# msotoodeh/curve25519

Measured on AMD Instinct MI355X. Metric: X25519 shared-key ops/sec (batch=2^20 per GPU, variable-base Montgomery ladder) [+ Ed25519 verifies/sec in `verify`], higher is better.
Workload: dtype u64

## Files before the change

### curve25519_amd/csrc/engine_verify.hip

```cpp
#include "engine_common.cuh"
#include "verify_check.cuh"

constexpr int FS_BLOCK = 256;
#ifndef C25519_VW_WAVES
#define C25519_VW_WAVES 2
#endif
#ifndef C25519_WALK_BLOCK
#define C25519_WALK_BLOCK C25519_ED_BLOCK
#endif
constexpr int WALK_BLOCK = C25519_WALK_BLOCK;
#ifndef C25519_VD_WAVES
#define C25519_VD_WAVES 3
#endif

template <bool Strict = false>
C25519_DEV void verify_scalars_lane(const FastScratch& fs, const void* sig, const void* pk, const Msgs& msgs, size_t n, size_t i)
{
    u32 pkw[8], Rw[8], Sw[8], cols[SIGMA_WORDS], rho[5], tau[5], tau_neg;
    load32(pkw, pk, i);
    load32(Rw, sig, 2 * i);
    load32(Sw, sig, 2 * i + 1);
    const u32 lat_ok = ed_verify_fast_scalars(cols, rho, tau, tau_neg, pkw, Rw, Sw, msgs.ptr(i), msgs.len(i), fs.lat_cap_bits);
#pragma unroll
    for (int w = 0; w < SIGMA_WORDS; w++) fs.sigma[(size_t)w * n + i] = cols[w];
#pragma unroll
    for (int w = 0; w < 5; w++) { fs.rho[(size_t)w * n + i] = rho[w]; fs.tau[(size_t)w * n + i] = tau[w]; }
    const int top = lat_ok ? walk_top_digit(tau, rho) : 0;
    if (Strict) {
        load32(Rw, sig, 2 * i);
        load32(Sw, sig, 2 * i + 1);
        fs.flags[i] = (lat_ok & FLAG_FITS) | (tau_neg & FLAG_TAU_NEG) | ((u32)top << 8) | strict_pair_flags(Rw, Sw);
    } else
        fs.flags[i] = (lat_ok & FLAG_FITS) | (tau_neg & FLAG_TAU_NEG) | ((u32)top << 8);
}


template <bool Strict>
C25519_DEV void verify_fast_scalars(const FastScratch& fs, const void* sig, const void* pk, const Msgs& msgs, size_t n)
{
    const size_t i = (size_t)blockIdx.x * FS_BLOCK + threadIdx.x;
    if (i == 0) fs.slow_count[0] = fs.slow_count[1] = fs.slow_count[2] = 0;
    if (i >= n) return;
    verify_scalars_lane<Strict>(fs, sig, pk, msgs, n, i);
}

__global__ void __launch_bounds__(FS_BLOCK) k_ed25519_verify_fast_scalars(FastScratch fs, const void* sig, const void* pk,
                                                                          Msgs msgs, size_t n)
{
    verify_fast_scalars<false>(fs, sig, pk, msgs, n);
}

__global__ void __launch_bounds__(FS_BLOCK) k_ed25519_verify_fast_scalars_strict(FastScratch fs, const void* sig, const void* pk,
                                                                                 Msgs msgs, size_t n)
{
    verify_fast_scalars<true>(fs, sig, pk, msgs, n);
}

template <bool Strict>
C25519_DEV void verify_fast_points(FastScratch fs, const void* sig, const void* pk, size_t n, int* verdict)
{
    const size_t j = (size_t)blockIdx.x * ED_BLOCK + threadIdx.x;
    if (j >= 2 * n) return;
    const bool is_r = j >= n;
    const size_t e = is_r ? j - n : j;
    u32 w[8];
    if (is_r) load32(w, sig, 2 * e); else load32(w, pk, e);
    const u32 f = fs.flags[e];
    const u32 tau_neg = (f & FLAG_TAU_NEG) ? 0xffffffffu : 0u;
    fe X, Y;
    const u32 ok = ed_verify_fast_decode(X, Y, w, is_r ? 0xffffffffu : 0u, tau_neg) & (Strict && !is_r ? ~strict_reject_key(w) : 0xffffffffu);
    if (!is_r) {
        const bool is_long = ((f >> 8) & 63u) > 32u;
        const u32 pos = is_long ? (u32)n - 1u - atomicAdd(fs.slow_count + 2, 1u) : atomicAdd(fs.slow_count + 1, 1u);
        fs.order[pos] = (u32)e;
    }
    if (is_r) {
        if (ok) atomicOr(&fs.flags[e], FLAG_R_OK);
    } else if (Strict) {
        const u32 add = strict_key_flags(f, ok);
        atomicOr(&fs.flags[e], add);
        if (add & FLAG_REJECT) verdict[e] = 0;
        else if (add & FLAG_SLOW) fs.slow_list[atomicAdd(fs.slow_count, 1u)] = (u32)e;
    } else if (ok && (f & FLAG_FITS)) {
        atomicOr(&fs.flags[e], FLAG_KEY_OK);
    } else {
        atomicOr(&fs.flags[e], ok ? FLAG_KEY_OK | FLAG_SLOW : FLAG_SLOW);
        fs.slow_list[atomicAdd(fs.slow_count, 1u)] = (u32)e;
    }
    wtable_build(fs.tables + e * FAST_TABLE_WORDS + (is_r ? WTABLE_WORDS : 0), X, Y);
}

__global__ void __launch_bounds__(ED_BLOCK, C25519_VD_WAVES) k_ed25519_verify_fast_points(FastScratch fs, const void* sig, const void* pk,
                                                                                          size_t n)
{
    verify_fast_points<false>(fs, sig, pk, n, nullptr);
}

__global__ void __launch_bounds__(ED_BLOCK, C25519_VD_WAVES) k_ed25519_verify_fast_points_strict(FastScratch fs, const void* sig,
                                                                                                 const void* pk, size_t n, int* verdict)
{
    verify_fast_points<true>(fs, sig, pk, n, verdict);
}

__global__ void __launch_bounds__(WALK_BLOCK, C25519_VW_WAVES) k_ed25519_verify_fast_walk(FastScratch fs, int* verdict, size_t n,
                                                                                        const u32* __restrict__ g_tbl)
{
    __shared__ __attribute__((aligned(16))) u32 lds_tbl[SC_TBL_WORDS];
    lds_stage_words(lds_tbl, g_tbl + SC_TBL_OFFSET, SC_TBL_WORDS);
    const size_t lane = (size_t)blockIdx.x * WALK_BLOCK + threadIdx.x;
    const size_t i = lane < n ? fs.order[lane] : n;
    const u32 f = i < n ? fs.flags[i] : FLAG_SLOW;
    const bool walks = !(f & FLAG_SLOW);
    int top = walks ? (int)((f >> 8) & 63u) : 0;
#pragma unroll
    for (int o = 32; o >= 1; o >>= 1) {
        const int other = __shfl_xor(top, o);
        top = other > top ? other : top;
    }
    top = __builtin_amdgcn_readfirstlane(top);
    if (!walks) return;
    const u32* tq = fs.tables + i * FAST_TABLE_WORDS;
    const WalkScalars sc{ fs.sigma, fs.tau, fs.rho, n, i };
    const u32 neutral = ge_walk_is_neutral(sc, tq, tq + WTABLE_WORDS, lds_tbl, top < 8 ? 8 : top);
    verdict[i] = (neutral & f & FLAG_R_OK) ? 1 : 0;
}

__global__ void __launch_bounds__(ED_BLOCK, C25519_VD_WAVES) k_ed25519_verify_quad_prep(FastScratch fs, const void* sig, const void* pk,
                                                                                         Msgs msgs, size_t n, unsigned scalar_blocks)
{
    static_assert(FS_BLOCK == ED_BLOCK, "one workgroup shape for both roles");
    if (blockIdx.x < scalar_blocks) {
        const size_t i = (size_t)blockIdx.x * FS_BLOCK + threadIdx.x;
        if (i == 0) fs.slow_count[0] = fs.slow_count[1] = fs.slow_count[2] = 0;
        if (i >= n) return;
        verify_scalars_lane(fs, sig, pk, msgs, n, i);
        return;
    }
    const size_t j = (size_t)(blockIdx.x - scalar_blocks) * ED_BLOCK + threadIdx.x;
    if (j >= 2 * n) return;
    const bool is_r = j >= n;
    const size_t e = is_r ? j - n : j;
    u32 w[8];
    if (is_r) load32(w, sig, 2 * e); else load32(w, pk, e);
    fe X, Y;
    const u32 ok = ed_verify_fast_decode(X, Y, w, is_r ? 0xffffffffu : 0u, 0u);
    fs.pflags[j] = ok;
    wtable_build(fs.tables + e * FAST_TABLE_WORDS + (is_r ? WTABLE_WORDS : 0), X, Y);
}

__global__ void __launch_bounds__(ED_BLOCK, C25519_VD_WAVES) k_ed25519_verify_quad_prep_strict(FastScratch fs, const void* sig, const void* pk,
                                                                                                Msgs msgs, size_t n, unsigned scalar_blocks)
{
    if (blockIdx.x < scalar_blocks) {
        const size_t i = (size_t)blockIdx.x * FS_BLOCK + threadIdx.x;
        if (i == 0) fs.slow_count[0] = fs.slow_count[1] = fs.slow_count[2] = 0;
        if (i >= n) return;
        verify_scalars_lane<true>(fs, sig, pk, msgs, n, i);
        return;
    }
    const size_t j = (size_t)(blockIdx.x - scalar_blocks) * ED_BLOCK + threadIdx.x;
    if (j >= 2 * n) return;
    const bool is_r = j >= n;
    const size_t e = is_r ? j - n : j;
    u32 w[8];
    if (is_r) load32(w, sig, 2 * e); else load32(w, pk, e);
    fe X, Y;
    const u32 ok = ed_verify_fast_decode(X, Y, w, is_r ? 0xffffffffu : 0u, 0u) & (is_r ? 0xffffffffu : ~strict_reject_key(w));
    fs.pflags[j] = ok;
    wtable_build(fs.tables + e * FAST_TABLE_WORDS + (is_r ? WTABLE_WORDS : 0), X, Y);
}

constexpr int QW_BLOCK = 256;
__global__ void __launch_bounds__(QW_BLOCK) __attribute__((amdgpu_waves_per_eu(1, 2)))
k_ed25519_verify_quad_walk(FastScratch fs, int* verdict, size_t n, const u32* __restrict__ g_tbl)
{
    __shared__ __attribute__((aligned(16))) u32 lds_tbl[SC_TBL_WORDS];
    lds_stage_words(lds_tbl, g_tbl + SC_TBL_OFFSET, SC_TBL_WORDS);
    const size_t i = (size_t)blockIdx.x * (QW_BLOCK / 4) + (threadIdx.x >> 2);
    const u32 f = i < n ? fs.flags[i] : 0u;
    const u32 key_ok = i < n ? fs.pflags[i] : 0u, r_ok = i < n ? fs.pflags[n + i] : 0u;
    const bool walks = (f & FLAG_FITS) && key_ok;
    int top = walks ? (int)((f >> 8) & 63u) : 0;
#pragma unroll
    for (int o = 32; o >= 1; o >>= 1) {
        const int other = __shfl_xor(top, o);
        top = other > top ? other : top;
    }
    top = __builtin_amdgcn_readfirstlane(top);
    const quad::Roles R = quad::roles();
    if (!walks) {
        if (i < n && R.is0) fs.slow_list[atomicAdd(fs.slow_count, 1u)] = (u32)i;
        return;
    }
    const u32* tq = fs.tables + i * FAST_TABLE_WORDS;
    const WalkScalars sc{ fs.sigma, fs.tau, fs.rho, n, i };
    const u32 q_flip = (f & FLAG_TAU_NEG) ? 0xffffffffu : 0u;
    const u32 neutral = quad::walk_is_neutral(sc, tq, tq + WTABLE_WORDS, lds_tbl, top < 8 ? 8 : top, R, q_flip);
    if (R.is0) verdict[i] = (neutral & r_ok) ? 1 : 0;
}

__global__ void __launch_bounds__(QW_BLOCK) __attribute__((amdgpu_waves_per_eu(1, 2)))
k_ed25519_verify_quad_walk_strict(FastScratch fs, int* verdict, size_t n, const u32* __restrict__ g_tbl)
{
    __shared__ __attribute__((aligned(16))) u32 lds_tbl[SC_TBL_WORDS];
    lds_stage_words(lds_tbl, g_tbl + SC_TBL_OFFSET, SC_TBL_WORDS);
    const size_t i = (size_t)blockIdx.x * (QW_BLOCK / 4) + (threadIdx.x >> 2);
    const u32 f = i < n ? fs.flags[i] : 0u;
    const u32 key_ok = i < n ? fs.pflags[i] : 0u, r_ok = i < n ? fs.pflags[n + i] : 0u;
    const bool rejected = i < n && ((f & FLAG_REJECT) || !key_ok);
    const bool walks = !rejected && (f & FLAG_FITS);
    int top = walks ? (int)((f >> 8) & 63u) : 0;
#pragma unroll
    for (int o = 32; o >= 1; o >>= 1) {
        const int other = __shfl_xor(top, o);
        top = other > top ? other : top;
    }
    top = __builtin_amdgcn_readfirstlane(top);
    const quad::Roles R = quad::roles();
    if (!walks) {
        if (rejected && R.is0) verdict[i] = 0;
        else if (i < n && R.is0) fs.slow_list[atomicAdd(fs.slow_count, 1u)] = (u32)i;
        return;
    }
    const u32* tq = fs.tables + i * FAST_TABLE_WORDS;
    const WalkScalars sc{ fs.sigma, fs.tau, fs.rho, n, i };
    const u32 q_flip = (f & FLAG_TAU_NEG) ? 0xffffffffu : 0u;
    const u32 neutral = quad::walk_is_neutral(sc, tq, tq + WTABLE_WORDS, lds_tbl, top < 8 ? 8 : top, R, q_flip);
    if (R.is0) verdict[i] = (neutral & r_ok) ? 1 : 0;
}

__global__ void __launch_bounds__(192) __attribute__((amdgpu_waves_per_eu(1, 2)))
k_ed25519_verify_one_per_group(FastScratch fs, int* verdict, const void* sig, const void* pk, Msgs msgs, size_t n,
                               const u32* __restrict__ g_tbl)
{
    __shared__ __attribute__((aligned(16))) u32 lds_all[coop::V3_LDS_WORDS];
    __shared__ u32 park[40], hand[4];
    if (blockIdx.x >= n) return;
    coop::verify_three_waves(lds_all, park, hand, fs, verdict, sig, pk, msgs, n, blockIdx.x, g_tbl);
}

__global__ void __launch_bounds__(192) __attribute__((amdgpu_waves_per_eu(1, 2)))
k_ed25519_verify_one_per_group_strict(FastScratch fs, int* verdict, const void* sig, const void* pk, Msgs msgs, size_t n,
                                      const u32* __restrict__ g_tbl)
{
    __shared__ __attribute__((aligned(16))) u32 lds_all[coop::V3_LDS_WORDS];
    __shared__ u32 park[40], hand[4];
    if (blockIdx.x >= n) return;
    coop::verify_three_waves<true>(lds_all, park, hand, fs, verdict, sig, pk, msgs, n, blockIdx.x, g_tbl);
}

__global__ void __launch_bounds__(ED_BLOCK, 2) k_ed25519_verify_slow(FastScratch fs, int* verdict, const void* sig, const void* pk,
                                                                     Msgs msgs, const u32* __restrict__ g_tbl, DoneWord done)
{
    const u32 count = *fs.slow_count;
    if (blockIdx.x == 0 && threadIdx.x == 0) {
        *fs.slow_report = count;
        if (count == 0) signal_done(done);
    }
    if ((size_t)blockIdx.x * ED_BLOCK >= count) return;
    __shared__ __attribute__((aligned(16))) u32 lds_tbl[PA_WORDS * 256];
    lds_stage_words(lds_tbl, g_tbl + REF_TBL_OFFSET, REF_TBL_WORDS);
    const size_t k = (size_t)blockIdx.x * ED_BLOCK + threadIdx.x;
    if (k >= count) return;
    const size_t i = fs.slow_list[k];
    u32 pkw[8], Rw[8], Sw[8];
    load32(pkw, pk, i);
    load32(Rw, sig, 2 * i);
    load32(Sw, sig, 2 * i + 1);
    verdict[i] = ed_verify_reference_order(pkw, Rw, Sw, msgs.ptr(i), msgs.len(i), fs.tables + i * FAST_TABLE_WORDS, lds_tbl);
    if (k == 0) signal_done(done);
}


template <bool Scale8>
C25519_DEV void verify_scalars_lane_zip215(const FastScratch& fs, const void* sig, const void* pk, const Msgs& msgs, size_t n, size_t i)
{
    u32 pkw[8], Rw[8], Sw[8], cols[SIGMA_WORDS], rho[5], tau[5], tau_neg;
    load32(pkw, pk, i);
    load32(Rw, sig, 2 * i);
    load32(Sw, sig, 2 * i + 1);
    const u32 lat_ok = ed_verify_zip215_scalars(cols, rho, tau, tau_neg, pkw, Rw, Sw, msgs.ptr(i), msgs.len(i), fs.lat_cap_bits, Scale8);
#pragma unroll
    for (int w = 0; w < SIGMA_WORDS; w++) fs.sigma[(size_t)w * n + i] = cols[w];
#pragma unroll
    for (int w = 0; w < 5; w++) { fs.rho[(size_t)w * n + i] = rho[w]; fs.tau[(size_t)w * n + i] = tau[w]; }
    const int top = lat_ok ? walk_top_digit(tau, rho) : 0;
    load32(Sw, sig, 2 * i + 1);
    fs.flags[i] = (lat_ok & FLAG_FITS) | (tau_neg & FLAG_TAU_NEG) | ((u32)top << 8) | zip215_pair_flags(Sw);
}

__global__ void __launch_bounds__(FS_BLOCK) k_ed25519_verify_fast_scalars_zip215(FastScratch fs, const void* sig, const void* pk,
                                                                                 Msgs msgs, size_t n)
{
    const size_t i = (size_t)blockIdx.x * FS_BLOCK + threadIdx.x;
    if (i == 0) fs.slow_count[0] = fs.slow_count[1] = fs.slow_count[2] = 0;
    if (i >= n) return;
    verify_scalars_lane_zip215<true>(fs, sig, pk, msgs, n, i);
}

__global__ void __launch_bounds__(ED_BLOCK, C25519_VD_WAVES) k_ed25519_verify_fast_points_zip215(FastScratch fs, const void* sig,
                                                                                                 const void* pk, size_t n, int* verdict)
{
    const size_t j = (size_t)blockIdx.x * ED_BLOCK + threadIdx.x;
    if (j >= 2 * n) return;
    const bool is_r = j >= n;
    const size_t e = is_r ? j - n : j;
    u32 w[8];
    if (is_r) load32(w, sig, 2 * e); else load32(w, pk, e);
    const u32 f = fs.flags[e];
    fe X, Y;
    const u32 ok = ed_zip215_decode(X, Y, w, (is_r || !(f & FLAG_TAU_NEG)) ? 0xffffffffu : 0u);
    if (!is_r) {
        const bool is_long = ((f >> 8) & 63u) > 33u;
        const u32 pos = is_long ? (u32)n - 1u - atomicAdd(fs.slow_count + 2, 1u) : atomicAdd(fs.slow_count + 1, 1u);
        fs.order[pos] = (u32)e;
    }
    if (is_r) {
        if (ok) atomicOr(&fs.flags[e], FLAG_R_OK);
    } else {
        const u32 add = strict_key_flags(f, ok);
        atomicOr(&fs.flags[e], add);
        if (add & FLAG_REJECT) verdict[e] = 0;
        else if (add & FLAG_SLOW) fs.slow_list[atomicAdd(fs.slow_count, 1u)] = (u32)e;
    }
    wtable_build(fs.tables + e * FAST_TABLE_WORDS + (is_r ? WTABLE_WORDS : 0), X, Y);
}

__global__ void __launch_bounds__(ED_BLOCK, C25519_VD_WAVES) k_ed25519_verify_quad_prep_zip215(FastScratch fs, const void* sig, const void* pk,
                                                                                                Msgs msgs, size_t n, unsigned scalar_blocks)
{
    if (blockIdx.x < scalar_blocks) {
        const size_t i = (size_t)blockIdx.x * FS_BLOCK + threadIdx.x;
        if (i == 0) fs.slow_count[0] = fs.slow_count[1] = fs.slow_count[2] = 0;
        if (i >= n) return;
        verify_scalars_lane_zip215<false>(fs, sig, pk, msgs, n, i);
        return;
    }
    const size_t j = (size_t)(blockIdx.x - scalar_blocks) * ED_BLOCK + threadIdx.x;
    if (j >= 2 * n) return;
    const bool is_r = j >= n;
    const size_t e = is_r ? j - n : j;
    u32 w[8];
    if (is_r) load32(w, sig, 2 * e); else load32(w, pk, e);
    fe X, Y;
    const u32 ok = ed_zip215_decode(X, Y, w, 0xffffffffu);
    fs.pflags[j] = ok;
    wtable_build(fs.tables + e * FAST_TABLE_WORDS + (is_r ? WTABLE_WORDS : 0), X, Y);
}

__global__ void __launch_bounds__(QW_BLOCK) __attribute__((amdgpu_waves_per_eu(1, 2)))
k_ed25519_verify_quad_walk_zip215(FastScratch fs, int* verdict, size_t n, const u32* __restrict__ g_tbl)
{
    __shared__ __attribute__((aligned(16))) u32 lds_tbl[SC_TBL_WORDS];
    lds_stage_words(lds_tbl, g_tbl + SC_TBL_OFFSET, SC_TBL_WORDS);
    const size_t i = (size_t)blockIdx.x * (QW_BLOCK / 4) + (threadIdx.x >> 2);
    const u32 f = i < n ? fs.flags[i] : 0u;
    const u32 key_ok = i < n ? fs.pflags[i] : 0u, r_ok = i < n ? fs.pflags[n + i] : 0u;
    const bool rejected = i < n && ((f & FLAG_REJECT) || !key_ok || !r_ok);
    const bool walks = !rejected && (f & FLAG_FITS);
    int top = walks ? (int)((f >> 8) & 63u) : 0;
#pragma unroll
    for (int o = 32; o >= 1; o >>= 1) {
        const int other = __shfl_xor(top, o);
        top = other > top ? other : top;
    }
    top = __builtin_amdgcn_readfirstlane(top);
    const quad::Roles R = quad::roles();
    if (!walks) {
        if (rejected && R.is0) verdict[i] = 0;
        else if (i < n && R.is0) fs.slow_list[atomicAdd(fs.slow_count, 1u)] = (u32)i;
        return;
    }
    const u32* tq = fs.tables + i * FAST_TABLE_WORDS;
    const WalkScalars sc{ fs.sigma, fs.tau, fs.rho, n, i };
    const u32 q_flip = (f & FLAG_TAU_NEG) ? 0xffffffffu : 0u;
    const u32 neutral = quad::walk_is_neutral<true>(sc, tq, tq + WTABLE_WORDS, lds_tbl, top < 8 ? 8 : top, R, q_flip);
    if (R.is0) verdict[i] = neutral ? 1 : 0;
}

__global__ void __launch_bounds__(192) __attribute__((amdgpu_waves_per_eu(1, 2)))
k_ed25519_verify_one_per_group_zip215(FastScratch fs, int* verdict, const void* sig, const void* pk, Msgs msgs, size_t n,
                                      const u32* __restrict__ g_tbl)
{
    __shared__ __attribute__((aligned(16))) u32 lds_all[coop::V3_LDS_WORDS];
    __shared__ u32 park[40], hand[4];
    if (blockIdx.x >= n) return;
    coop::verify_three_waves<false, true>(lds_all, park, hand, fs, verdict, sig, pk, msgs, n, blockIdx.x, g_tbl);
}

__global__ void __launch_bounds__(ED_BLOCK, 2) k_ed25519_verify_slow_zip215(FastScratch fs, int* verdict, const void* sig, const void* pk,
                                                                            Msgs msgs, const u32* __restrict__ g_tbl, DoneWord done)
{
    const u32 count = *fs.slow_count;
    if (blockIdx.x == 0 && threadIdx.x == 0) {
        *fs.slow_report = count;
        if (count == 0) signal_done(done);
    }
    if ((size_t)blockIdx.x * ED_BLOCK >= count) return;
    __shared__ __attribute__((aligned(16))) u32 lds_tbl[PA_WORDS * 256];
    lds_stage_words(lds_tbl, g_tbl + REF_TBL_OFFSET, REF_TBL_WORDS);
    const size_t k = (size_t)blockIdx.x * ED_BLOCK + threadIdx.x;
    if (k >= count) return;
    const size_t i = fs.slow_list[k];
    u32 pkw[8], Rw[8], Sw[8];
    load32(pkw, pk, i);
    load32(Rw, sig, 2 * i);
    load32(Sw, sig, 2 * i + 1);
    verdict[i] = ed_verify_zip215_reference_order(pkw, Rw, Sw, msgs.ptr(i), msgs.len(i), fs.tables + i * FAST_TABLE_WORDS, lds_tbl);
    if (k == 0) signal_done(done);
}

namespace {

constexpr size_t VERIFY_TABLE_WORDS = FAST_TABLE_WORDS > QTABLE_LIMB_WORDS ? FAST_TABLE_WORDS : QTABLE_LIMB_WORDS;
static_assert(FAST_TABLE_WORDS % 32 == 0 && VERIFY_TABLE_WORDS % 32 == 0, "per-lane tables must keep their rows 128-byte aligned");
inline size_t verify_scalar_words(size_t n) { return round_up(SIGMA_WORDS * n, 4) + 2 * round_up(5 * n, 4) + 5 * round_up(n, 4) + 4; }
inline size_t verify_scratch_bytes(size_t n)
{
    return (n * VERIFY_TABLE_WORDS + proj_words(n) + verify_scalar_words(n)) * sizeof(u32);
}

struct LastVerify { const u32* count = nullptr; hipStream_t stream = nullptr; int device = -1; unsigned long generation = 0; };
thread_local LastVerify tl_last_verify;

template <typename MakeFin>
int verify_run(const void* sig, const void* pk, Msgs msgs, size_t n, hipStream_t stream, int* verdict, bool fast, MakeFin make_fin,
               VerifyRules rules = RULES_PLAIN, bool last_in_call = true)
{
    const bool strict = rules == RULES_STRICT, zip215 = rules == RULES_ZIP215;
    const u32* tbl = nullptr;
    C25519_RC(base_tables(&tbl, nullptr));
    void* w = nullptr;
    c25519_host::WorkLease lease;
    C25519_RC(lease.acquire(&w, verify_scratch_bytes(n), stream));
    u32* tables = (u32*)w;
    const ProjScratch scr = carve_proj(tables + n * VERIFY_TABLE_WORDS, n);
    const unsigned grid = grid_for(n, ED_BLOCK);
    if (fast) {
        unsigned* report = nullptr;
        C25519_RC(tls().report_word_for(&report, stream));
        FastScratch fs;
        fs.tables = tables;
        fs.sigma = tables + n * VERIFY_TABLE_WORDS + proj_words(n);
        fs.rho = fs.sigma + round_up(SIGMA_WORDS * n, 4);
        fs.tau = fs.rho + round_up(5 * n, 4);
        fs.flags = fs.tau + round_up(5 * n, 4);
        fs.slow_list = fs.flags + round_up(n, 4);
        fs.order = fs.slow_list + round_up(n, 4);
        fs.slow_count = fs.order + round_up(n, 4);
        fs.pflags = fs.slow_count + 4;
        fs.slow_report = report;
        {
            const long cap = c25519_host::tunable_or(c25519_host::T_VERIFY_LAT_CAP_BITS, LAT_CAP_BITS);
            fs.lat_cap_bits = cap >= 100 && cap < LAT_CAP_BITS ? (int)cap : LAT_CAP_BITS;
        }
        if (!verify_quad_for(n) && verify_coop_for(n)) {
            C25519_TRY(hipMemsetAsync(fs.slow_count, 0, 3 * sizeof(u32), stream));
            note_shape(SHAPE_PER_GROUP, 192);
            (zip215 ? k_ed25519_verify_one_per_group_zip215 : strict ? k_ed25519_verify_one_per_group_strict : k_ed25519_verify_one_per_group)<<<(unsigned)n, 192, 0, stream>>>(
                fs, verdict, sig, pk, msgs, n, tbl);
            C25519_TRY(hipGetLastError());
        } else if (verify_quad_for(n)) {
            const unsigned sb = grid_for(n, FS_BLOCK);
            note_shape(SHAPE_QUAD, QW_BLOCK);
            (zip215 ? k_ed25519_verify_quad_prep_zip215 : strict ? k_ed25519_verify_quad_prep_strict : k_ed25519_verify_quad_prep)<<<sb + grid_for(2 * n, ED_BLOCK), ED_BLOCK, 0, stream>>>(
                fs, sig, pk, msgs, n, sb);
            C25519_TRY(hipGetLastError());
            (zip215 ? k_ed25519_verify_quad_walk_zip215 : strict ? k_ed25519_verify_quad_walk_strict : k_ed25519_verify_quad_walk)<<<grid_for(n, QW_BLOCK / 4), QW_BLOCK, 0, stream>>>(
                fs, verdict, n, tbl);
            C25519_TRY(hipGetLastError());
        } else {
            note_shape(SHAPE_LANE, WALK_BLOCK);
            (zip215 ? k_ed25519_verify_fast_scalars_zip215 : strict ? k_ed25519_verify_fast_scalars_strict : k_ed25519_verify_fast_scalars)<<<grid_for(n, FS_BLOCK), FS_BLOCK, 0, stream>>>(
                fs, sig, pk, msgs, n);
            C25519_TRY(hipGetLastError());
            if (zip215)
                k_ed25519_verify_fast_points_zip215<<<grid_for(2 * n, ED_BLOCK), ED_BLOCK, 0, stream>>>(fs, sig, pk, n, verdict);
            else if (strict)
                k_ed25519_verify_fast_points_strict<<<grid_for(2 * n, ED_BLOCK), ED_BLOCK, 0, stream>>>(fs, sig, pk, n, verdict);
            else
                k_ed25519_verify_fast_points<<<grid_for(2 * n, ED_BLOCK), ED_BLOCK, 0, stream>>>(fs, sig, pk, n);
            C25519_TRY(hipGetLastError());
            k_ed25519_verify_fast_walk<<<grid_for(n, WALK_BLOCK), WALK_BLOCK, 0, stream>>>(fs, verdict, n, tbl);
            C25519_TRY(hipGetLastError());
        }
        (zip215 ? k_ed25519_verify_slow_zip215 : k_ed25519_verify_slow)<<<grid, ED_BLOCK, 0, stream>>>(fs, verdict, sig, pk, msgs, tbl,
                                                                                                     last_in_call ? take_done_word(n) : DoneWord{ nullptr, 0 });
        C25519_TRY(hipGetLastError());
        tl_last_verify.count = report; tl_last_verify.stream = stream;
        tl_last_verify.generation = tls().generation;
        (void)hipGetDevice(&tl_last_verify.device);
        return lease.release();
    }
    tl_last_verify = LastVerify();
    note_shape(SHAPE_LANE_INVERT, ED_BLOCK);
    k_ed25519_verify_init<QTableLimbs><<<grid, ED_BLOCK, 0, stream>>>(pk, n, tables, VERIFY_TABLE_WORDS);
    C25519_TRY(hipGetLastError());
    k_ed25519_verify_check<QTableLimbs><<<grid, ED_BLOCK, 0, stream>>>(scr, sig, pk, msgs, n, tbl, tables, VERIFY_TABLE_WORDS);
    C25519_TRY(hipGetLastError());
    C25519_RC(launch_invert(scr, n, make_fin(scr), stream));
    return lease.release();
}

}

int c25519_engine::verify_dev(void* verdict, const void* sig, const void* pk, Msgs msgs, size_t n, hipStream_t stream, VerifyRules rules,
                              bool last_in_call)
{
    const bool fast = rules != RULES_PLAIN || c25519_host::tunable_or(c25519_host::T_VERIFY_REFERENCE_ORDER, 0) == 0;
    if (int rc = check_dev_args(n, { verdict, sig, pk })) return rc;
    if (n == 0) return 0;
    return verify_run(sig, pk, msgs, n, stream, (int*)verdict, fast,
                      [&](const ProjScratch& scr) { return FinishVerify{ scr.a, scr.b, sig, (int*)verdict, n, nullptr }; }, rules, last_in_call);
}

extern "C" {

size_t ed25519_VerifySignature_scratch_bytes(size_t n) { return verify_scratch_bytes(n); }

int c25519_amd_verify_point_dev(void* out, const void* sig, const void* pk, const void* msg, size_t msg_size, size_t n,
                                void* stream)
{
    C25519_API_CALL();
    if (!out || !sig || !pk || (!msg && msg_size)) return bad_arg("null pointer");
    if (int rc = check_dev_args(n, { out, sig, pk })) return rc;
    if (n == 0) return 0;
    return verify_run(sig, pk, fixed_msgs(msg, msg_size), n, (hipStream_t)stream, nullptr, false,
                      [&](const ProjScratch& scr) { return FinishPack{ scr.a, scr.b, out, n, 1, 0, nullptr, 0, 0 }; });
}

long c25519_amd_verify_last_slow_elements(void)
{
    C25519_API_CALL_OR(-1);
    const LastVerify& lv = tl_last_verify;
    int dev = -1;
    if (!lv.count || hipGetDevice(&dev) != hipSuccess || dev != lv.device) return -1;
    if (lv.generation != tls().generation) return -1;
    if (hipStreamSynchronize(lv.stream) != hipSuccess) return -1;
    u32 c = 0;
    if (hipMemcpy(&c, lv.count, sizeof c, hipMemcpyDeviceToHost) != hipSuccess) return -1;
    return (long)c;
}

int ed25519_VerifySignature_dev(void* verdict, const void* sig, const void* pk, const void* msg, size_t msg_size,
                                size_t n, void* stream)
{
    C25519_API_CALL();
    if (!verdict || !sig || !pk || (!msg && msg_size)) return bad_arg("null pointer");
    return verify_dev(verdict, sig, pk, fixed_msgs(msg, msg_size), n, (hipStream_t)stream, RULES_PLAIN);
}

int ed25519_VerifySignature_ragged_dev(void* verdict, const void* sig, const void* pk, const void* msgs,
                                       const uint64_t* offsets, size_t n, void* stream)
{
    C25519_API_CALL();
    if (!verdict || !sig || !pk || !offsets) return bad_arg("null pointer");
    return verify_dev(verdict, sig, pk, ragged_msgs(msgs, offsets), n, (hipStream_t)stream, RULES_PLAIN);
}

int ed25519_VerifySignature_strict_dev(void* verdict, const void* sig, const void* pk, const void* msg, size_t msg_size,
                                       size_t n, void* stream)
{
    C25519_API_CALL();
    if (!verdict || !sig || !pk || (!msg && msg_size)) return bad_arg("null pointer");
    return verify_dev(verdict, sig, pk, fixed_msgs(msg, msg_size), n, (hipStream_t)stream, RULES_STRICT);
}

int ed25519_VerifySignature_strict_ragged_dev(void* verdict, const void* sig, const void* pk, const void* msgs,
                                              const uint64_t* offsets, size_t n, void* stream)
{
    C25519_API_CALL();
    if (!verdict || !sig || !pk || !offsets) return bad_arg("null pointer");
    return verify_dev(verdict, sig, pk, ragged_msgs(msgs, offsets), n, (hipStream_t)stream, RULES_STRICT);
}

int ed25519_VerifySignature_zip215_dev(void* verdict, const void* sig, const void* pk, const void* msg, size_t msg_size,
                                       size_t n, void* stream)
{
    C25519_API_CALL();
    if (!verdict || !sig || !pk || (!msg && msg_size)) return bad_arg("null pointer");
    return verify_dev(verdict, sig, pk, fixed_msgs(msg, msg_size), n, (hipStream_t)stream, RULES_ZIP215);
}

int ed25519_VerifySignature_zip215_ragged_dev(void* verdict, const void* sig, const void* pk, const void* msgs,
                                              const uint64_t* offsets, size_t n, void* stream)
{
    C25519_API_CALL();
    if (!verdict || !sig || !pk || !offsets) return bad_arg("null pointer");
    return verify_dev(verdict, sig, pk, ragged_msgs(msgs, offsets), n, (hipStream_t)stream, RULES_ZIP215);
}

}
```

### curve25519_amd/csrc/verify_fast.cuh

```cuda
#pragma once
#include "ge25519.cuh"
#include "lanes.cuh"
#include "sc25519.cuh"
#include "sha512.cuh"

namespace c25519 {

constexpr int LAT_CAP_BITS = 158;
#ifndef C25519_LAT_COUNT
#define C25519_LAT_COUNT(what)
#endif
constexpr int LAT_LEHMER_STOP = 128;
constexpr int LAT_R = 8, LAT_T = 6;

template <int W>
C25519_DEV int bitlen_words(const u32 (&a)[W])
{
    int n = 0;
#pragma unroll
    for (int i = 0; i < W; i++) n = a[i] ? 32 * i + (32 - __builtin_clz(a[i])) : n;
    return n;
}
C25519_DEV int bitlen64(u64 x) { return x ? 64 - __builtin_clzll(x) : 0; }
template <int W>
// ... 490 lines not shown
    for (int i = 0; i < 10; i++) q.v[i] = p_ymx[i * SC_ROWS];
    fe_mul(a, a, q);
    fe_add(b, S.Y, S.X);
#pragma unroll
    for (int i = 0; i < 10; i++) q.v[i] = p_ypx[i * SC_ROWS];
    fe_mul(b, b, q);
    fe_sub(e, b, a);
    fe_add(h, b, a);
#pragma unroll
    for (int i = 0; i < 10; i++) q.v[i] = tbl[(20 + i) * SC_ROWS + r];
    fe_neg(a, q);
    fe_select(q, neg, a, q);
    fe_mul(a, S.T, q);
    fe_add(b, S.Z, S.Z);
    fe_sub(f, b, a);
    fe_add(g, b, a);
    fe_mul(S.X, f, e);
    if (need_t) fe_mul(S.T, e, h);
    fe_mul(S.Z, f, g);
    fe_mul(S.Y, g, h);
}

C25519_DEV void ge_store_pe_row(u32* row, const ge_ext& S)
{
    fe t, a;
    fe_add(t, S.Y, S.X);  fe_carry32(a, t);  store_field(row, a);
    fe_sub(t, S.Y, S.X);  fe_carry32(a, t);  store_field(row + 8, a);
    fe_mul(a, S.T, fe_const(K_2D));          store_field(row + 16, a);
    fe_add(t, S.Z, S.Z);  fe_carry32(a, t);  store_field(row + 24, a);
}

C25519_DEV void wtable_build(u32* rows, const fe& x, const fe& y)
{
    ge_ext S;
    row_store_neutral(rows);
    S.X = x; S.Y = y;
    fe_mul(S.T, x, y);
    fe_set_u32(S.Z, 1);
    ge_store_pe_row(rows + ROW_WORDS, S);
#pragma unroll 1
    for (int step = 0; step < 7; step++) {
        if (step == 4 || step == 6) {
            ge_pe pe;
            row_load_pe(pe, rows + (step == 4 ? 2 : 4) * ROW_WORDS);
            ge_from_pe(S, pe);
        }
        if (step & 1) ge_add_pe_row<true>(S, rows + ROW_WORDS, 0u);
        else ge_double<true>(S);
        ge_store_pe_row(rows + ((0x8547632u >> (4 * step)) & 15u) * ROW_WORDS, S);
    }
}

C25519_DEV void qtable_build_streamed(u32* rows, ge_ext& Q)
{
    row_store_neutral(rows);
    ge_store_pe_row(rows + ROW_WORDS, Q);
#pragma unroll 1
    for (int blk = 1; blk < 4; blk++) {
#pragma unroll 1
        for (int i = 0; i < 63; i++) ge_double<false>(Q);
        ge_double<true>(Q);
        const int top = 1 << blk;
        ge_store_pe_row(rows + top * ROW_WORDS, Q);
#pragma unroll 1
        for (int s = 1; s <= top; s++) {
            ge_pe pe;
            row_load_pe(pe, rows + top * ROW_WORDS);
            ge_from_pe(Q, pe);
            if (s == top) break;
            ge_add_pe_row<true>(Q, rows + s * ROW_WORDS, 0u);
            ge_store_pe_row(rows + (top + s) * ROW_WORDS, Q);
        }
    }
}

C25519_DEV void ge_poly_mult_streamed(ge_ext& S, u32 (&s)[8], u32 (&h)[8], const u32* rows, const u32* lds_tbl)
{
    {
        ge_pe pe;
        row_load_pe(pe, rows + fold4_next(h, false) * ROW_WORDS);
        ge_from_pe(S, pe);
    }
#pragma unroll 1
    for (int i = 1; i < 32; i++) {
        ge_double(S);
        ge_add_pe_row<false>(S, rows + fold4_next(h, false) * ROW_WORDS, 0u);
    }
#pragma unroll 1
    for (int i = 32; i < 64; i++) {
        ge_double(S);
        ge_add_pa_lds(S, lds_tbl, fold8_next(s), true);
        ge_add_pe_row<false>(S, rows + fold4_next(h, true) * ROW_WORDS, 0u);
    }
}

C25519_DEV int ed_verify_reference_order(const u32 (&pkw)[8], const u32 (&Rw)[8], u32 (&Sw)[8], const uint8_t* msg, size_t len,
                                         u32* lane_table, const u32* lds_tbl, u32* enc_out = nullptr)
{
    u32 h[8], enc[8], xw[8], yw[8];
    {
        ge_ext Q;
        ed_decode_neg_key(Q, pkw);
        qtable_build_streamed(lane_table, Q);
    }
    ed_hram(h, Rw, pkw, msg, len);
    sc_mod(h);
    ge_ext T;
    ge_poly_mult_streamed(T, Sw, h, lane_table, lds_tbl);
    ge_to_affine_words(xw, yw, T);
    ge_pack(enc, xw, yw);
    u32 diff = 0;
#pragma unroll
    for (int j = 0; j < 8; j++) diff |= enc[j] ^ Rw[j];
    if (enc_out) {
#pragma unroll
        for (int j = 0; j < 8; j++) enc_out[j] = enc[j];
    }
    return diff == 0 ? 1 : 0;
}

struct WalkScalars {
    const u32 *sigma_cols, *tau, *rho;
    size_t n, i;
    C25519_DEV u32 tau_word(int w) const { return tau[(size_t)w * n + i]; }
    C25519_DEV u32 rho_word(int w) const { return rho[(size_t)w * n + i]; }
    C25519_DEV u32 sigma_word(int w) const { return sigma_cols[(size_t)w * n + i]; }
};

C25519_DEV u32 ge_walk_is_neutral(const WalkScalars& sc, const u32* tq, const u32* tr, const u32* lds_tbl, int top)
{
    ge_ext S;
    {
        ge_pe pe;
        u32 neg;
        const u32 m = signed16_of(neg, sc.tau_word(top >> 3), top & 7);
        row_load_pe(pe, tq + m * ROW_WORDS);
        pe_cond_neg(pe, neg);
        ge_from_pe(S, pe);
        const u32 m2 = signed16_of(neg, sc.rho_word(top >> 3), top & 7);
        ge_add_pe_row<false>(S, tr + m2 * ROW_WORDS, neg);
    }
#pragma unroll 1
    for (int i = top - 1; i >= 0; i--) {
        const u32 tw = sc.tau_word(i >> 3), rw = sc.rho_word(i >> 3);
        u32 negq, negr;
        packed_row rq, rr;
        row_fetch(rq, tq + signed16_of(negq, tw, i & 7) * ROW_WORDS);
        row_fetch(rr, tr + signed16_of(negr, rw, i & 7) * ROW_WORDS);
        if (i >= SC_ROUNDS) {
#pragma unroll 1
            for (int j = 0; j < 3; j++) ge_double<false>(S);
            ge_double<true>(S);
        } else {
            u64 cols = (u64)sc.sigma_word(2 * i) | ((u64)sc.sigma_word(2 * i + 1) << 32);
#pragma unroll 1
            for (int j = 0; j < 4; j++) {
                ge_double<true>(S);
                if (4 * i + 3 - j < SC_COLS)
                    ge_add_pa_comb(S, lds_tbl, (u32)cols & 0xffffu, j == 3);
                cols >>= 16;
            }
        }
        ge_add_pe_regs<true>(S, rq, negq);
        ge_add_pe_regs<false>(S, rr, negr);
    }
    u32 xw[8], dw[8], acc = 0;
    fe d;
    fe_sub(d, S.Y, S.Z);
    fe_to_words(xw, S.X);
    fe_to_words(dw, d);
#pragma unroll
    for (int i = 0; i < 8; i++) acc |= xw[i] | dw[i];
    return acc == 0 ? 0xffffffffu : 0u;
}

C25519_DEV u32 ed_verify_fast_scalars(u32 (&sigma_cols)[SIGMA_WORDS], u32 (&rho)[5], u32 (&tau)[5], u32& tau_negative, const u32 (&pkw)[8],
                                      const u32 (&Rw)[8], const u32 (&Sw)[8], const uint8_t* msg, size_t len, int cap_bits = LAT_CAP_BITS)
{
    u32 h[8], sigma[8];
    {
        u32 le[16];
        u64 pre[8], dg[8];
        sha512_words_from_le32(pre, Rw);
        sha512_words_from_le32(pre + 4, pkw);
        sha512_prefixed<8>(dg, pre, msg, len);
        sha512_digest_le_words(le, dg);
        sc_reduce512(h, le);
        sc_mod(h);
    }
    const u32 lat_ok = sc_lattice_short(rho, tau, tau_negative, h, cap_bits);
    sc_mul_short(sigma, rho, Sw);
    sc_comb_columns(sigma_cols, sigma);
    u32 b[5];
    bias_signed16(b, rho);
#pragma unroll
    for (int i = 0; i < 5; i++) rho[i] = b[i];
    bias_signed16(b, tau);
#pragma unroll
    for (int i = 0; i < 5; i++) tau[i] = b[i];
    return lat_ok;
}

C25519_DEV u32 ed_verify_zip215_scalars(u32 (&sigma_cols)[SIGMA_WORDS], u32 (&rho)[5], u32 (&tau)[5], u32& tau_negative, const u32 (&pkw)[8],
                                        const u32 (&Rw)[8], const u32 (&Sw)[8], const uint8_t* msg, size_t len, int cap_bits, bool scale8)
{
    if (!scale8) return ed_verify_fast_scalars(sigma_cols, rho, tau, tau_negative, pkw, Rw, Sw, msg, len, cap_bits);
    u32 h[8], sigma[8];
    ed_hram(h, Rw, pkw, msg, len);
    sc_mod(h);
    const u32 lat_ok = sc_lattice_short(rho, tau, tau_negative, h, cap_bits - 3);
#pragma unroll
    for (int i = 4; i >= 0; i--) {
        rho[i] = (rho[i] << 3) | (i ? rho[i - 1] >> 29 : 0u);
        tau[i] = (tau[i] << 3) | (i ? tau[i - 1] >> 29 : 0u);
    }
    sc_mul_short(sigma, rho, Sw);
    sc_comb_columns(sigma_cols, sigma);
    u32 b[5];
    bias_signed16(b, rho);
#pragma unroll
    for (int i = 0; i < 5; i++) rho[i] = b[i];
    bias_signed16(b, tau);
#pragma unroll
    for (int i = 0; i < 5; i++) tau[i] = b[i];
    return lat_ok;
}

C25519_DEV u32 ed_verify_fast_decode(fe& X, fe& Y, const u32 (&w)[8], u32 is_r, u32 tau_negative)
{
    u32 yw[8], cw[8];
#pragma unroll
    for (int i = 0; i < 8; i++) yw[i] = w[i];
    const u32 sign = yw[7] >> 31;
    yw[7] &= 0x7fffffffu;
    fe_from_words(Y, yw);
    const u32 parity = sign ^ (~is_r & 1u);
    u32 ok = ge_calc_x_checked(X, Y, parity);
    fe_to_words(cw, Y);
    u32 diff = 0;
#pragma unroll
    for (int i = 0; i < 8; i++) diff |= cw[i] ^ yw[i];
    fe_to_words(cw, X);
    const u32 canonical = (diff == 0 && ((cw[0] ^ parity) & 1u) == 0) ? 0xffffffffu : 0u;
    ok &= ~is_r | canonical;
    fe t;
    fe_neg(t, X);
    fe_carry32(t, t);
    fe_select(X, is_r | tau_negative, t, X);
    return ok;
}

C25519_DEV u32 ed_zip215_decode(fe& X, fe& Y, const u32 (&w)[8], u32 negate)
{
    u32 yw[8];
#pragma unroll
    for (int i = 0; i < 8; i++) yw[i] = w[i];
    const u32 sign = yw[7] >> 31;
    yw[7] &= 0x7fffffffu;
    fe_from_words(Y, yw);
    const u32 ok = ge_calc_x_checked(X, Y, sign);
    fe t;
    fe_neg(t, X);
    fe_carry32(t, t);
    fe_select(X, negate, t, X);
    return ok;
}

C25519_DEV int ed_verify_zip215_reference_order(const u32 (&pkw)[8], const u32 (&Rw)[8], u32 (&Sw)[8], const uint8_t* msg, size_t len,
                                                u32* lane_table, const u32* lds_tbl)
{
    u32 h[8];
    {
        ge_ext Q;
        ed_decode_neg_key(Q, pkw);
        qtable_build_streamed(lane_table, Q);
    }
    ed_hram(h, Rw, pkw, msg, len);
    sc_mod(h);
    ge_ext T;
    ge_poly_mult_streamed(T, Sw, h, lane_table, lds_tbl);
#pragma unroll 1
    for (int j = 0; j < 3; j++) ge_double<false>(T);
    ge_ext R;
    const u32 r_ok = ed_zip215_decode(R.X, R.Y, Rw, 0u);
    fe_set_u32(R.Z, 1);
#pragma unroll 1
    for (int j = 0; j < 3; j++) ge_double<false>(R);
    fe a, b;
    u32 aw[8], bw[8], acc = 0;
    fe_mul(a, T.X, R.Z);
    fe_mul(b, R.X, T.Z);
    fe_sub(a, a, b);
    fe_to_words(aw, a);
    fe_mul(a, T.Y, R.Z);
    fe_mul(b, R.Y, T.Z);
    fe_sub(a, a, b);
    fe_to_words(bw, a);
#pragma unroll
    for (int i = 0; i < 8; i++) acc |= aw[i] | bw[i];
    return (acc == 0 && r_ok) ? 1 : 0;
}


}
```

Measured before the change: 130.7 million.

## Use wide comb base-point tables in the fast Ed25519 verify walk

Swaps the sigma*B part of the verify walk from an LDS-staged small table for a wide comb table held in global memory. Sigma is recoded into packed 16-bit columns and consumed in the last steps of the walk, so the main loop over tau/rho digits now stops at level 2 instead of 8. The point is to drop doublings and the per-block LDS staging. In exchange the kernel fetches larger rows with gather-style global loads, and the plain, strict and zip215 scalar kernels are merged into one templated path. The X25519 ladder metric is not touched; only the verify path is.

```diff
diff --git a/curve25519_amd/csrc/engine_verify.hip b/curve25519_amd/csrc/engine_verify.hip
--- a/curve25519_amd/csrc/engine_verify.hip
+++ b/curve25519_amd/csrc/engine_verify.hip
@@ -35,25 +35,41 @@
 }
 
 
-template <bool Strict>
+template <int RULES>
 C25519_DEV void verify_fast_scalars(const FastScratch& fs, const void* sig, const void* pk, const Msgs& msgs, size_t n)
 {
     const size_t i = (size_t)blockIdx.x * FS_BLOCK + threadIdx.x;
     if (i == 0) fs.slow_count[0] = fs.slow_count[1] = fs.slow_count[2] = 0;
     if (i >= n) return;
-    verify_scalars_lane<Strict>(fs, sig, pk, msgs, n, i);
+    u32 pkw[8], Rw[8], Sw[8], cols[WSIGMA_WORDS], rho[5], tau[5], tau_neg;
+    load32(pkw, pk, i);
+    load32(Rw, sig, 2 * i);
+    load32(Sw, sig, 2 * i + 1);
+    const u32 lat_ok = ed_verify_scalars_wide<RULES == 2>(cols, rho, tau, tau_neg, pkw, Rw, Sw, msgs.ptr(i), msgs.len(i), fs.lat_cap_bits);
+#pragma unroll
+    for (int w = 0; w < WSIGMA_WORDS; w++) fs.sigma[(size_t)w * n + i] = cols[w];
+#pragma unroll
+    for (int w = 0; w < 5; w++) { fs.rho[(size_t)w * n + i] = rho[w]; fs.tau[(size_t)w * n + i] = tau[w]; }
+    const int top = lat_ok ? walk_top_digit(tau, rho) : 0;
+    u32 f = (lat_ok & FLAG_FITS) | (tau_neg & FLAG_TAU_NEG) | ((u32)top << 8);
+    if (RULES) {
+        if (RULES == 1) load32(Rw, sig, 2 * i);
+        load32(Sw, sig, 2 * i + 1);
+        f |= RULES == 1 ? strict_pair_flags(Rw, Sw) : zip215_pair_flags(Sw);
+    }
+    fs.flags[i] = f;
 }
 
 __global__ void __launch_bounds__(FS_BLOCK) k_ed25519_verify_fast_scalars(FastScratch fs, const void* sig, const void* pk,
                                                                           Msgs msgs, size_t n)
 {
-    verify_fast_scalars<false>(fs, sig, pk, msgs, n);
+    verify_fast_scalars<0>(fs, sig, pk, msgs, n);
 }
 
 __global__ void __launch_bounds__(FS_BLOCK) k_ed25519_verify_fast_scalars_strict(FastScratch fs, const void* sig, const void* pk,
                                                                                  Msgs msgs, size_t n)
 {
-    verify_fast_scalars<true>(fs, sig, pk, msgs, n);
+    verify_fast_scalars<1>(fs, sig, pk, msgs, n);
 }
 
 template <bool Strict>
@@ -103,10 +119,8 @@
 }
 
 __global__ void __launch_bounds__(WALK_BLOCK, C25519_VW_WAVES) k_ed25519_verify_fast_walk(FastScratch fs, int* verdict, size_t n,
-                                                                                        const u32* __restrict__ g_tbl)
-{
-    __shared__ __attribute__((aligned(16))) u32 lds_tbl[SC_TBL_WORDS];
-    lds_stage_words(lds_tbl, g_tbl + SC_TBL_OFFSET, SC_TBL_WORDS);
+                                                                                        const u32* __restrict__ g_wide)
+{
     const size_t lane = (size_t)blockIdx.x * WALK_BLOCK + threadIdx.x;
     const size_t i = lane < n ? fs.order[lane] : n;
     const u32 f = i < n ? fs.flags[i] : FLAG_SLOW;
@@ -121,7 +135,7 @@
     if (!walks) return;
     const u32* tq = fs.tables + i * FAST_TABLE_WORDS;
     const WalkScalars sc{ fs.sigma, fs.tau, fs.rho, n, i };
-    const u32 neutral = ge_walk_is_neutral(sc, tq, tq + WTABLE_WORDS, lds_tbl, top < 8 ? 8 : top);
+    const u32 neutral = ge_walk_wide_is_neutral(sc, tq, tq + WTABLE_WORDS, g_wide, top < 2 ? 2 : top);
     verdict[i] = (neutral & f & FLAG_R_OK) ? 1 : 0;
 }
 
@@ -292,10 +306,7 @@
 __global__ void __launch_bounds__(FS_BLOCK) k_ed25519_verify_fast_scalars_zip215(FastScratch fs, const void* sig, const void* pk,
                                                                                  Msgs msgs, size_t n)
 {
-    const size_t i = (size_t)blockIdx.x * FS_BLOCK + threadIdx.x;
-    if (i == 0) fs.slow_count[0] = fs.slow_count[1] = fs.slow_count[2] = 0;
-    if (i >= n) return;
-    verify_scalars_lane_zip215<true>(fs, sig, pk, msgs, n, i);
+    verify_fast_scalars<2>(fs, sig, pk, msgs, n);
 }
 
 __global__ void __launch_bounds__(ED_BLOCK, C25519_VD_WAVES) k_ed25519_verify_fast_points_zip215(FastScratch fs, const void* sig,
@@ -428,8 +439,9 @@
                VerifyRules rules = RULES_PLAIN, bool last_in_call = true)
 {
     const bool strict = rules == RULES_STRICT, zip215 = rules == RULES_ZIP215;
-    const u32* tbl = nullptr;
+    const u32 *tbl = nullptr, *wide = nullptr;
     C25519_RC(base_tables(&tbl, nullptr));
+    if (fast) C25519_RC(wide_tables(&wide));
     void* w = nullptr;
     c25519_host::WorkLease lease;
     C25519_RC(lease.acquire(&w, verify_scratch_bytes(n), stream));
@@ -481,7 +493,7 @@
             else
                 k_ed25519_verify_fast_points<<<grid_for(2 * n, ED_BLOCK), ED_BLOCK, 0, stream>>>(fs, sig, pk, n);
             C25519_TRY(hipGetLastError());
-            k_ed25519_verify_fast_walk<<<grid_for(n, WALK_BLOCK), WALK_BLOCK, 0, stream>>>(fs, verdict, n, tbl);
+            k_ed25519_verify_fast_walk<<<grid_for(n, WALK_BLOCK), WALK_BLOCK, 0, stream>>>(fs, verdict, n, wide);
             C25519_TRY(hipGetLastError());
         }
         (zip215 ? k_ed25519_verify_slow_zip215 : k_ed25519_verify_slow)<<<grid, ED_BLOCK, 0, stream>>>(fs, verdict, sig, pk, msgs, tbl,
diff --git a/curve25519_amd/csrc/verify_fast.cuh b/curve25519_amd/csrc/verify_fast.cuh
--- a/curve25519_amd/csrc/verify_fast.cuh
+++ b/curve25519_amd/csrc/verify_fast.cuh
@@ -816,4 +816,141 @@
 }
 
 
-}
+constexpr int WSIGMA_WORDS = WB_COLS / 2;
+static_assert(WSIGMA_WORDS <= SIGMA_WORDS && WB_NT == 4 && WB_STEP == 5, "the columns live in sigma's scratch words; a level is two words");
+
+template <bool SCALE8>
+C25519_DEV u32 ed_verify_scalars_wide(u32 (&sigma_cols)[WSIGMA_WORDS], u32 (&rho)[5], u32 (&tau)[5], u32& tau_negative, const u32 (&pkw)[8],
+                                      const u32 (&Rw)[8], const u32 (&Sw)[8], const uint8_t* msg, size_t len, int cap_bits)
+{
+    u32 h[8], sigma[8];
+    ed_hram(h, Rw, pkw, msg, len);
+    sc_mod(h);
+    const u32 lat_ok = sc_lattice_short(rho, tau, tau_negative, h, SCALE8 ? cap_bits - 3 : cap_bits);
+    if (SCALE8) {
+#pragma unroll
+        for (int i = 4; i >= 0; i--) {
+            rho[i] = (rho[i] << 3) | (i ? rho[i - 1] >> 29 : 0u);
+            tau[i] = (tau[i] << 3) | (i ? tau[i - 1] >> 29 : 0u);
+        }
+    }
+    sc_mul_short(sigma, rho, Sw);
+    u32 c[WB_COLS];
+    wb_columns(c, 1, sigma);
+#pragma unroll
+    for (int i = 0; i < WSIGMA_WORDS; i++) sigma_cols[i] = c[2 * i] | (c[2 * i + 1] << 16);
+    u32 b[5];
+    bias_signed16(b, rho);
+#pragma unroll
+    for (int i = 0; i < 5; i++) rho[i] = b[i];
+    bias_signed16(b, tau);
+#pragma unroll
+    for (int i = 0; i < 5; i++) tau[i] = b[i];
+    return lat_ok;
+}
+
+struct wide_row { uint4 q[6]; u32 neg; };
+C25519_DEV void wide_fetch(wide_row& r, const u32* __restrict__ tbl, u32 c)
+{
+    r.neg = ((c >> (WB_TEETH - 1)) & 1u) - 1u;
+    const uint4* p = reinterpret_cast<const uint4*>(tbl + (size_t)((c ^ r.neg) & (u32)(WB_ROWS - 1)) * WB_ROW_WORDS);
+#pragma unroll
+    for (int i = 0; i < 6; i++) r.q[i] = p[i];
+}
+C25519_DEV void wide_field(fe& f, const wide_row& r, int k, int k_neg)
+{
+    const uint4 a = r.q[2 * k], b = r.q[2 * k + 1], c = r.q[2 * k_neg], d = r.q[2 * k_neg + 1];
+    const u32 wa[8] = { a.x, a.y, a.z, a.w, b.x, b.y, b.z, b.w }, wb[8] = { c.x, c.y, c.z, c.w, d.x, d.y, d.z, d.w };
+    u32 w[8];
+#pragma unroll
+    for (int i = 0; i < 8; i++) w[i] = r.neg ? wb[i] : wa[i];
+    fe_from_words(f, w);
+}
+C25519_DEV void ge_add_wide_regs(ge_ext& S, const wide_row& r, bool need_t)
+{
+    fe q, a, b, e, f, g, h;
+    fe_sub(a, S.Y, S.X);
+    wide_field(q, r, 1, 0);
+    fe_mul(a, a, q);
+    fe_add(b, S.Y, S.X);
+    wide_field(q, r, 0, 1);
+    fe_mul(b, b, q);
+    fe_sub(e, b, a);
+    fe_add(h, b, a);
+    wide_field(q, r, 2, 2);
+    fe_neg(a, q);
+    fe_select(q, r.neg, a, q);
+    fe_mul(a, S.T, q);
+    fe_add(b, S.Z, S.Z);
+    fe_sub(f, b, a);
+    fe_add(g, b, a);
+    fe_mul(S.X, f, e);
+    if (need_t) fe_mul(S.T, e, h);
+    fe_mul(S.Z, f, g);
+    fe_mul(S.Y, g, h);
+}
+
+C25519_DEV u32 ge_walk_wide_is_neutral(const WalkScalars& sc, const u32* tq, const u32* tr, const u32* __restrict__ g_wide, int top)
+{
+    ge_ext S;
+    {
+        ge_pe pe;
+        u32 neg;
+        const u32 m = signed16_of(neg, sc.tau_word(top >> 3), top & 7);
+        row_load_pe(pe, tq + m * ROW_WORDS);
+        pe_cond_neg(pe, neg);
+        ge_from_pe(S, pe);
+        const u32 m2 = signed16_of(neg, sc.rho_word(top >> 3), top & 7);
+        ge_add_pe_row<false>(S, tr + m2 * ROW_WORDS, neg);
+    }
+#pragma unroll 1
+    for (int i = top - 1; i >= 2; i--) {
+        const u32 tw = sc.tau_word(i >> 3), rw = sc.rho_word(i >> 3);
+        u32 negq, negr;
+        packed_row rq, rr;
+        row_fetch(rq, tq + signed16_of(negq, tw, i & 7) * ROW_WORDS);
+        row_fetch(rr, tr + signed16_of(negr, rw, i & 7) * ROW_WORDS);
+#pragma unroll 1
+        for (int j = 0; j < 3; j++) ge_double<false>(S);
+        ge_double<true>(S);
+        ge_add_pe_regs<true>(S, rq, negq);
+        ge_add_pe_regs<false>(S, rr, negr);
+    }
+    const u32 tw = sc.tau_word(0), rw = sc.rho_word(0);
+    auto column = [&](int s) -> u32 { return (sc.sigma_word(s >> 1) >> (16 * (s & 1))) & 0xffffu; };
+    wide_row next;
+    wide_fetch(next, g_wide, column(0));
+#pragma unroll 1
+    for (int m = 0; m < WB_STEP; m++) {
+        if (m == 0) {
+#pragma unroll 1
+            for (int j = 0; j < 3; j++) ge_double<false>(S);
+        }
+        ge_double<true>(S);
+#pragma unroll 1
+        for (int t = 0; t < WB_NT; t++) {
+            const wide_row cur = next;
+            const int s1 = m * WB_NT + t + 1;
+            if (s1 < WB_COLS) wide_fetch(next, g_wide + (size_t)(s1 & (WB_NT - 1)) * WB_ROWS * WB_ROW_WORDS, column(s1));
+            ge_add_wide_regs(S, cur, t != WB_NT - 1 || m == 0 || m == WB_STEP - 1);
+        }
+        if (m == 0 || m == WB_STEP - 1) {
+            const int i = m ? 0 : 1;
+            u32 negq, negr;
+            const u32 mq = signed16_of(negq, tw, i), mr = signed16_of(negr, rw, i);
+            ge_add_pe_row<true>(S, tq + mq * ROW_WORDS, negq);
+            if (m == 0) ge_add_pe_row<false>(S, tr + mr * ROW_WORDS, negr);
+            else ge_add_pe_row<false>(S, tr + mr * ROW_WORDS, negr);
+        }
+    }
+    u32 xw[8], dw[8], acc = 0;
+    fe d;
+    fe_sub(d, S.Y, S.Z);
+    fe_to_words(xw, S.X);
+    fe_to_words(dw, d);
+#pragma unroll
+    for (int i = 0; i < 8; i++) acc |= xw[i] | dw[i];
+    return acc == 0 ? 0xffffffffu : 0u;
+}
+
+}
```

Measured after the change: 130.9 million (median of 2 runs). No clear change (+0.2%).
